# SnakeOnex/vit-is-all-you-need

Hardware: AMD Instinct MI355X
Metric: images/sec ViT-B/16 224px bf16 fwd+bwd (higher is better)
Workload: dtype bf16; 1 GPU; ViT-B/16 224x224 bf16 forward+loss+backward, batch 256 per GPU (BASELINE configs[1]; configs[2] at 8 GPUs), random-init weights, 197 tokens, 79.44 M params; global_batch=256, parallelism=dp1

## Files before the change

### vit-is-all-you-need_amd/csrc/attention.hip

```cpp
#include "common.h"

namespace {

constexpr int DH = 64;
constexpr int MAX_N = 512;
constexpr int MAX_N_LONG = 16384;
constexpr float NEG_BIG = -1.0e30f;

typedef LDS_AS bf16x4* lds_bf16x4_ptr;

__device__ __forceinline__ int swz(int row) { return (((row >> 1) & 1) << 2) | ((row >> 3) & 3); }

__device__ __forceinline__ void stage_tile(const __bf16* __restrict__ g, int ld, int N, int npad, char* lds, int wave, int lane, int nwaves = 4) {
  const int pieces = npad / 8;
  for (int pc = wave; pc < pieces; pc += nwaves) {
    const int row = pc * 8 + (lane >> 3);
    const int logical = (lane & 7) ^ swz(row);
    const int grow = min(row, N - 1);
    glds16(g + (size_t)grow * ld + logical * 8, lds + pc * 1024);
  }
}

__device__ __forceinline__ bf16x8 row_frag(const char* tile, int T, int kk, int lane) {
  const int rr = lane & 31;
// ... 361 lines not shown
  char* oimg = smem + 2 * npad * 128 + wave * 2048;
  const __bf16* qbase = a.qkv + (size_t)b * N * D3 + hh * DH;
  stage_tile(qbase + D, D3, N, npad, ktile, wave, lane, 8);
  stage_tile(qbase + 2 * D, D3, N, npad, vtile, wave, lane, 8);
  const int qb = (wave + head) & 7;
  const bool active = qb < nt;
  bf16x8 qf[4];
  load_lane_frags(qbase, D3, N, (active ? qb : 0) * 32, lane, qf);
  asm volatile("s_waitcnt vmcnt(0)" ::: "memory");
#pragma unroll
  for (int kk = 0; kk < 4; ++kk) asm volatile("" : "+v"(qf[kk]));
  __syncthreads();
  if (!active) return;
  const float c = a.scale_log2e;
  const int q0 = qb * 32;
  const int qrow = q0 + (lane & 31);
  float m = NEG_BIG, l = 0.f;
  f32x16 oacc[2];
#pragma unroll
  for (int dt = 0; dt < 2; ++dt)
#pragma unroll
    for (int r = 0; r < 16; ++r) oacc[dt][r] = 0.f;
#pragma unroll 1
  for (int T = 0; T < NKT; ++T) {
    f32x16 st;
#pragma unroll
    for (int r = 0; r < 16; ++r) st[r] = 0.f;
#pragma unroll
    for (int kk = 0; kk < 4; ++kk) st = __builtin_amdgcn_mfma_f32_32x32x16_bf16(row_frag(ktile, T, kk, lane), qf[kk], st, 0, 0, 0);
    if (32 * T + 32 > N) {
#pragma unroll
      for (int r = 0; r < 16; ++r)
        if (!(32 * T + acc_row(r, lane) < N)) st[r] = NEG_BIG;
    }
    float mt = max16(st);
    mt = fmaxf(mt, __shfl_xor(mt, 32, 64));
    const float mn = fmaxf(m, mt);
    const float alpha = fast_exp2((m - mn) * c);
    m = mn;
    const float mc = mn * c;
    float lt = 0.f;
#pragma unroll
    for (int r = 0; r < 16; ++r) {
      const float pexp = fast_exp2(__builtin_fmaf(st[r], c, -mc));
      lt += pexp;
      st[r] = pexp;
    }
    l = l * alpha + lt;
    if (T > 0) {
#pragma unroll
      for (int dt = 0; dt < 2; ++dt)
#pragma unroll
        for (int r = 0; r < 16; ++r) oacc[dt][r] *= alpha;
    }
#pragma unroll
    for (int sidx = 0; sidx < 2; ++sidx) {
      const bf16x8 pf = acc_to_frag(st, sidx);
#pragma unroll
      for (int dt = 0; dt < 2; ++dt)
        oacc[dt] = __builtin_amdgcn_mfma_f32_32x32x16_bf16(tr_frag(vtile, T, sidx, dt, lane), pf, oacc[dt], 0, 0, 0);
    }
  }
  l += __shfl_xor(l, 32, 64);
  const float mc = m * c;
  const float inv = 1.0f / l;
  if constexpr (RES)
    store_rows_T_lds2k<true>(a.o + (size_t)b * N * D + hh * DH, D, N, q0, lane, oacc, inv, oimg, a.resid_in + (size_t)b * N * D + hh * DH,
                             a.resid_out + (size_t)b * N * D + hh * DH, D);
  else
    store_rows_T_lds2k(a.o + (size_t)b * N * D + hh * DH, D, N, q0, lane, oacc, inv, oimg);
  if (lane < 32 && qrow < N) a.lse2[((size_t)b * a.H + hh) * N + qrow] = mc + log2f(l);
}

template <bool DROP, bool CAUSAL>
__global__ __launch_bounds__(256, 2) void attn_bwd_dq_kernel(const AttnArgs a) {
  extern __shared__ __attribute__((aligned(16))) char smem[];
  const int lane = threadIdx.x & 63, wave = __builtin_amdgcn_readfirstlane(threadIdx.x >> 6);
  const int b = blockIdx.x / a.H, hh = blockIdx.x % a.H;
  const int N = a.N, D3 = 3 * a.H * DH, D = a.H * DH;
  const int nt = (N + 31) / 32, npad = nt * 32;
  char* ktile = smem;
  char* vtile = smem + npad * 128;
  char* oimg = smem + 2 * npad * 128 + wave * 4096;
  const __bf16* qbase = a.qkv + (size_t)b * N * D3 + hh * DH;
  stage_tile(qbase + D, D3, N, npad, ktile, wave, lane);
  stage_tile(qbase + 2 * D, D3, N, npad, vtile, wave, lane);
  asm volatile("s_waitcnt vmcnt(0)" ::: "memory");
  __syncthreads();

  const float c = a.scale_log2e;
  const __bf16* obase = a.o + (size_t)b * N * D + hh * DH;
  const __bf16* dobase = a.d_o + (size_t)b * N * D + hh * DH;
  float csum_q = 0.f;
  for (int qb = (wave + blockIdx.x) & 3; qb < nt; qb += 4) {
    const int q0 = qb * 32;
    const int qrow = q0 + (lane & 31);
    bf16x8 qf[4], dof[4], of[4];
    load_lane_frags(qbase, D3, N, q0, lane, qf);
    load_lane_frags(dobase, D, N, q0, lane, dof);
    load_lane_frags(obase, D, N, q0, lane, of);
    float delta = 0.f;
#pragma unroll
    for (int kk = 0; kk < 4; ++kk)
#pragma unroll
      for (int j = 0; j < 8; ++j) delta += (float)dof[kk][j] * (float)of[kk][j];
    delta += __shfl_xor(delta, 32, 64);
    const size_t stat = ((size_t)b * a.H + hh) * N + min(qrow, N - 1);
    const float lse2 = a.lse2[stat];
    if (lane < 32 && qrow < N) a.delta[stat] = delta;

    f32x16 dq[2];
#pragma unroll
    for (int dt = 0; dt < 2; ++dt)
#pragma unroll
      for (int r = 0; r < 16; ++r) dq[dt][r] = 0.f;
    const int t_end = CAUSAL ? min(nt, qb + 1) : nt;
    for (int T = 0; T < t_end; ++T) {
      f32x16 s, dp;
#pragma unroll
      for (int r = 0; r < 16; ++r) { s[r] = 0.f; dp[r] = 0.f; }
#pragma unroll
      for (int kk = 0; kk < 4; ++kk) {
        s = __builtin_amdgcn_mfma_f32_32x32x16_bf16(row_frag(ktile, T, kk, lane), qf[kk], s, 0, 0, 0);
        dp = __builtin_amdgcn_mfma_f32_32x32x16_bf16(row_frag(vtile, T, kk, lane), dof[kk], dp, 0, 0, 0);
      }
#pragma unroll
      for (int r = 0; r < 16; ++r) {
        const float pexp = fast_exp2(__builtin_fmaf(s[r], c, -lse2));
        float dpr = dp[r];
        if constexpr (DROP) dpr *= attn_keep(a, blockIdx.x, min(qrow, N - 1), min(32 * T + acc_row(r, lane), N - 1));
        s[r] = pexp * (dpr - delta);
      }
      if (32 * T + 32 > N || (CAUSAL && T == qb)) {
#pragma unroll
        for (int r = 0; r < 16; ++r) {
          const int key = 32 * T + acc_row(r, lane);
          if (!(key < N && (!CAUSAL || key <= qrow))) s[r] = 0.f;
        }
      }
#pragma unroll
      for (int sidx = 0; sidx < 2; ++sidx) {
        const bf16x8 dsf = acc_to_frag(s, sidx);
#pragma unroll
        for (int dt = 0; dt < 2; ++dt)
          dq[dt] = __builtin_amdgcn_mfma_f32_32x32x16_bf16(tr_frag(ktile, T, sidx, dt, lane), dsf, dq[dt], 0, 0, 0);
      }
    }
    store_rows_T_lds(a.dqkv + (size_t)b * N * D3 + hh * DH, D3, N, q0, lane, dq, a.scale, oimg, a.dbias ? &csum_q : nullptr);
  }
  if (a.dbias) atomicAdd(a.dbias + hh * DH + lane, csum_q);
}

template <int NT>
__global__ __launch_bounds__(256, 2) void attn_bwd_dq_pipe_kernel(const AttnArgs a) {
  extern __shared__ __attribute__((aligned(16))) char smem[];
  const int lane = threadIdx.x & 63, wave = __builtin_amdgcn_readfirstlane(threadIdx.x >> 6);
  const int head = blockIdx.x;
  const int b = head / a.H, hh = head % a.H;
  const int N = a.N, D3 = 3 * a.H * DH, D = a.H * DH;
  constexpr int nt = NT, npad = NT * 32;
  char* ktile = smem;
  char* vtile = smem + npad * 128;
  char* oimg = smem + 2 * npad * 128 + wave * 4096;
  const __bf16* qbase = a.qkv + (size_t)b * N * D3 + hh * DH;
  stage_tile(qbase + D, D3, N, npad, ktile, wave, lane);
  stage_tile(qbase + 2 * D, D3, N, npad, vtile, wave, lane);
  const __bf16* obase = a.o + (size_t)b * N * D + hh * DH;
  const __bf16* dobase = a.d_o + (size_t)b * N * D + hh * DH;
  asm volatile("s_waitcnt vmcnt(0)" ::: "memory");
  __syncthreads();

  const float c = a.scale_log2e;
  float csum_q = 0.f;
  for (int qb = (wave + head) & 3; qb < nt; qb += 4) {
    const int q0 = qb * 32;
    const int qrow = q0 + (lane & 31);
    bf16x8 qf[4], dof[4];
    float delta = 0.f;
    {
      bf16x8 of[4];
      load_lane_frags(qbase, D3, N, q0, lane, qf);
      load_lane_frags(dobase, D, N, q0, lane, dof);
      load_lane_frags(obase, D, N, q0, lane, of);
#pragma unroll
      for (int kk = 0; kk < 4; ++kk)
#pragma unroll
        for (int j = 0; j < 8; ++j) delta += (float)dof[kk][j] * (float)of[kk][j];
    }
    delta += __shfl_xor(delta, 32, 64);
    const size_t stat = ((size_t)b * a.H + hh) * N + min(qrow, N - 1);
    const float lse2 = a.lse2[stat];
    if (lane < 32 && qrow < N) a.delta[stat] = delta;

    f32x16 dq[2];
#pragma unroll
    for (int dt = 0; dt < 2; ++dt)
#pragma unroll
      for (int r = 0; r < 16; ++r) dq[dt][r] = 0.f;
    bf16x8 kr[2][4], vr[2][4];
    f32x16 sb[2], dpb[2];
    auto products = [&](int buf) {
#pragma unroll
      for (int r = 0; r < 16; ++r) { sb[buf][r] = 0.f; dpb[buf][r] = 0.f; }
#pragma unroll
      for (int kk = 0; kk < 4; ++kk) {
        sb[buf] = __builtin_amdgcn_mfma_f32_32x32x16_bf16(kr[buf][kk], qf[kk], sb[buf], 0, 0, 0);
        dpb[buf] = __builtin_amdgcn_mfma_f32_32x32x16_bf16(vr[buf][kk], dof[kk], dpb[buf], 0, 0, 0);
      }
    };
#pragma unroll
    for (int kk = 0; kk < 4; ++kk) { kr[0][kk] = row_frag(ktile, 0, kk, lane); vr[0][kk] = row_frag(vtile, 0, kk, lane); }
    if (NT > 1) {
#pragma unroll
      for (int kk = 0; kk < 4; ++kk) { kr[1][kk] = row_frag(ktile, 1, kk, lane); vr[1][kk] = row_frag(vtile, 1, kk, lane); }
    }
    products(0);
#pragma unroll
    for (int T = 0; T < NT; ++T) {
      const int cur = T & 1, nxt = cur ^ 1;
      bf16x8 ktr[2][2];
#pragma unroll
      for (int sidx = 0; sidx < 2; ++sidx)
#pragma unroll
        for (int dt = 0; dt < 2; ++dt) ktr[sidx][dt] = tr_frag(ktile, T, sidx, dt, lane);
      __builtin_amdgcn_sched_barrier(0);
      if (T + 1 < NT) products(nxt);
      if (T + 2 < NT) {
#pragma unroll
        for (int kk = 0; kk < 4; ++kk) { kr[cur][kk] = row_frag(ktile, T + 2, kk, lane); vr[cur][kk] = row_frag(vtile, T + 2, kk, lane); }
      }
#pragma unroll
      for (int r = 0; r < 16; ++r) {
        const float pexp = fast_exp2(__builtin_fmaf(sb[cur][r], c, -lse2));
        sb[cur][r] = pexp * (dpb[cur][r] - delta);
      }
      if (T == NT - 1 && 32 * T + 32 > N) {
#pragma unroll
        for (int r = 0; r < 16; ++r)
          if (!(32 * T + acc_row(r, lane) < N)) sb[cur][r] = 0.f;
      }
#pragma unroll
      for (int sidx = 0; sidx < 2; ++sidx) {
        const bf16x8 dsf = acc_to_frag(sb[cur], sidx);
#pragma unroll
        for (int dt = 0; dt < 2; ++dt) dq[dt] = __builtin_amdgcn_mfma_f32_32x32x16_bf16(ktr[sidx][dt], dsf, dq[dt], 0, 0, 0);
      }
    }
    store_rows_T_lds(a.dqkv + (size_t)b * N * D3 + hh * DH, D3, N, q0, lane, dq, a.scale, oimg, a.dbias ? &csum_q : nullptr);
  }
  if (a.dbias) atomicAdd(a.dbias + hh * DH + lane, csum_q);
}

template <bool DROP, bool CAUSAL>
__global__ __launch_bounds__(256, 2) void attn_bwd_dkv_kernel(const AttnArgs a) {
  extern __shared__ __attribute__((aligned(16))) char smem[];
  const int lane = threadIdx.x & 63, wave = __builtin_amdgcn_readfirstlane(threadIdx.x >> 6);
  const int b = blockIdx.x / a.H, hh = blockIdx.x % a.H;
  const int N = a.N, D3 = 3 * a.H * DH, D = a.H * DH;
  const int nt = (N + 31) / 32, npad = nt * 32;
  char* qtile = smem;
  char* dotile = smem + npad * 128;
  float* lse_s = (float*)(smem + 2 * npad * 128);
  float* delta_s = lse_s + npad;
  char* oimg = smem + 2 * npad * 128 + 2 * npad * 4 + wave * 4096;
  const __bf16* qbase = a.qkv + (size_t)b * N * D3 + hh * DH;
  const __bf16* dobase = a.d_o + (size_t)b * N * D + hh * DH;
  stage_tile(qbase, D3, N, npad, qtile, wave, lane);
  stage_tile(dobase, D, N, npad, dotile, wave, lane);
  for (int i = threadIdx.x; i < npad; i += 256) {
    const size_t stat = ((size_t)b * a.H + hh) * N + min(i, N - 1);
    lse_s[i] = a.lse2[stat];
    delta_s[i] = a.delta[stat];
  }
  asm volatile("s_waitcnt vmcnt(0)" ::: "memory");
  __syncthreads();

  const float c = a.scale_log2e;
  float csum_k = 0.f, csum_v = 0.f;
  for (int kb = (wave + blockIdx.x) & 3; kb < nt; kb += 4) {
    const int k0 = kb * 32;
    const int krow = k0 + (lane & 31);
    bf16x8 kf[4], vf[4];
    load_lane_frags(qbase + D, D3, N, k0, lane, kf);
    load_lane_frags(qbase + 2 * D, D3, N, k0, lane, vf);
    f32x16 dk[2], dv[2];
#pragma unroll
    for (int dt = 0; dt < 2; ++dt)
#pragma unroll
      for (int r = 0; r < 16; ++r) { dk[dt][r] = 0.f; dv[dt][r] = 0.f; }
    const int t_beg = CAUSAL ? kb : 0;
    for (int T = t_beg; T < nt; ++T) {
      f32x16 s, dp;
#pragma unroll
      for (int r = 0; r < 16; ++r) { s[r] = 0.f; dp[r] = 0.f; }
#pragma unroll
      for (int kk = 0; kk < 4; ++kk) {
        s = __builtin_amdgcn_mfma_f32_32x32x16_bf16(row_frag(qtile, T, kk, lane), kf[kk], s, 0, 0, 0);
        dp = __builtin_amdgcn_mfma_f32_32x32x16_bf16(row_frag(dotile, T, kk, lane), vf[kk], dp, 0, 0, 0);
      }
      f32x16 pmat;
#pragma unroll
      for (int u = 0; u < 4; ++u) {
        const int qr = 32 * T + 8 * u + 4 * (lane >> 5);
        const f32x4 lse4 = *(const f32x4*)(lse_s + qr);
        const f32x4 del4 = *(const f32x4*)(delta_s + qr);
#pragma unroll
        for (int i = 0; i < 4; ++i) {
          const int r = 4 * u + i;
          const float pexp = fast_exp2(__builtin_fmaf(s[r], c, -lse4[i]));
          float keep = 1.0f;
          if constexpr (DROP) keep = attn_keep(a, blockIdx.x, min(qr + i, N - 1), min(krow, N - 1));
          pmat[r] = pexp * keep;
          s[r] = pexp * (dp[r] * keep - del4[i]);
        }
        if (32 * T + 32 > N || k0 + 32 > N || (CAUSAL && T == kb)) {
#pragma unroll
          for (int i = 0; i < 4; ++i) {
            const int r = 4 * u + i, query = qr + i;
            if (!(query < N && krow < N && (!CAUSAL || krow <= query))) { pmat[r] = 0.f; s[r] = 0.f; }
          }
        }
      }
#pragma unroll
      for (int sidx = 0; sidx < 2; ++sidx) {
        const bf16x8 pf = acc_to_frag(pmat, sidx);
        const bf16x8 dsf = acc_to_frag(s, sidx);
#pragma unroll
        for (int dt = 0; dt < 2; ++dt) {
          dv[dt] = __builtin_amdgcn_mfma_f32_32x32x16_bf16(tr_frag(dotile, T, sidx, dt, lane), pf, dv[dt], 0, 0, 0);
          dk[dt] = __builtin_amdgcn_mfma_f32_32x32x16_bf16(tr_frag(qtile, T, sidx, dt, lane), dsf, dk[dt], 0, 0, 0);
        }
      }
    }
    __bf16* dbase = a.dqkv + (size_t)b * N * D3 + hh * DH;
    store_rows_T_lds(dbase + D, D3, N, k0, lane, dk, a.scale, oimg, a.dbias ? &csum_k : nullptr);
    store_rows_T_lds(dbase + 2 * D, D3, N, k0, lane, dv, 1.0f, oimg, a.dbias ? &csum_v : nullptr);
  }
  if (a.dbias) {
    atomicAdd(a.dbias + D + hh * DH + lane, csum_k);
    atomicAdd(a.dbias + 2 * D + hh * DH + lane, csum_v);
  }
}

template <int NT>
__global__ __launch_bounds__(256, 2) void attn_bwd_dkv_pipe_kernel(const AttnArgs a) {
  extern __shared__ __attribute__((aligned(16))) char smem[];
  const int lane = threadIdx.x & 63, wave = __builtin_amdgcn_readfirstlane(threadIdx.x >> 6);
  const int head = blockIdx.x;
  const int b = head / a.H, hh = head % a.H;
  const int N = a.N, D3 = 3 * a.H * DH, D = a.H * DH;
  constexpr int nt = NT, npad = NT * 32;
  char* qtile = smem;
  char* dotile = smem + npad * 128;
  float* lse_s = (float*)(smem + 2 * npad * 128);
  float* delta_s = lse_s + npad;
  char* oimg = smem + 2 * npad * 128 + 2 * npad * 4 + wave * 4096;
  const __bf16* qbase = a.qkv + (size_t)b * N * D3 + hh * DH;
  const __bf16* dobase = a.d_o + (size_t)b * N * D + hh * DH;
  stage_tile(qbase, D3, N, npad, qtile, wave, lane);
  stage_tile(dobase, D, N, npad, dotile, wave, lane);
  for (int i = threadIdx.x; i < npad; i += 256) {
    const size_t stat = ((size_t)b * a.H + hh) * N + min(i, N - 1);
    lse_s[i] = i < N ? a.lse2[stat] : 1.0e30f;
    delta_s[i] = a.delta[stat];
  }
  asm volatile("s_waitcnt vmcnt(0)" ::: "memory");
  __syncthreads();

  const float c = a.scale_log2e;
  float csum_k = 0.f, csum_v = 0.f;
  for (int kb = (wave + head) & 3; kb < nt; kb += 4) {
    const int k0 = kb * 32;
    bf16x8 kf[4], vf[4];
    load_lane_frags(qbase + D, D3, N, k0, lane, kf);
    load_lane_frags(qbase + 2 * D, D3, N, k0, lane, vf);
    f32x16 dk[2], dv[2];
#pragma unroll
    for (int dt = 0; dt < 2; ++dt)
#pragma unroll
      for (int r = 0; r < 16; ++r) { dk[dt][r] = 0.f; dv[dt][r] = 0.f; }
    bf16x8 qr[4], dor[4];
    f32x16 sb, dpb;
    auto products = [&]() {
#pragma unroll
      for (int r = 0; r < 16; ++r) { sb[r] = 0.f; dpb[r] = 0.f; }
#pragma unroll
      for (int kk = 0; kk < 4; ++kk) {
        sb = __builtin_amdgcn_mfma_f32_32x32x16_bf16(qr[kk], kf[kk], sb, 0, 0, 0);
        dpb = __builtin_amdgcn_mfma_f32_32x32x16_bf16(dor[kk], vf[kk], dpb, 0, 0, 0);
      }
    };
#pragma unroll
    for (int kk = 0; kk < 4; ++kk) { qr[kk] = row_frag(qtile, 0, kk, lane); dor[kk] = row_frag(dotile, 0, kk, lane); }
    products();
    if (NT > 1) {
#pragma unroll
      for (int kk = 0; kk < 4; ++kk) { qr[kk] = row_frag(qtile, 1, kk, lane); dor[kk] = row_frag(dotile, 1, kk, lane); }
    }
#pragma unroll
    for (int T = 0; T < NT; ++T) {
      bf16x8 dotr[2][2], qtr[2][2];
      f32x4 lse4[4], del4[4];
#pragma unroll
      for (int sidx = 0; sidx < 2; ++sidx)
#pragma unroll
        for (int dt = 0; dt < 2; ++dt) { dotr[sidx][dt] = tr_frag(dotile, T, sidx, dt, lane); qtr[sidx][dt] = tr_frag(qtile, T, sidx, dt, lane); }
      __builtin_amdgcn_sched_barrier(0);
#pragma unroll
      for (int u = 0; u < 4; ++u) {
        const int qr0 = 32 * T + 8 * u + 4 * (lane >> 5);
        lse4[u] = *(const f32x4*)(lse_s + qr0);
        del4[u] = *(const f32x4*)(delta_s + qr0);
      }
      f32x16 pmat;
#pragma unroll
      for (int u = 0; u < 4; ++u)
#pragma unroll
        for (int i = 0; i < 4; ++i) {
          const int r = 4 * u + i;
          const float pexp = fast_exp2(__builtin_fmaf(sb[r], c, -lse4[u][i]));
          pmat[r] = pexp;
          sb[r] = pexp * (dpb[r] - del4[u][i]);
        }
#pragma unroll
      for (int sidx = 0; sidx < 2; ++sidx) {
        const bf16x8 pf = acc_to_frag(pmat, sidx);
        const bf16x8 dsf = acc_to_frag(sb, sidx);
#pragma unroll
        for (int dt = 0; dt < 2; ++dt) {
          dv[dt] = __builtin_amdgcn_mfma_f32_32x32x16_bf16(dotr[sidx][dt], pf, dv[dt], 0, 0, 0);
          dk[dt] = __builtin_amdgcn_mfma_f32_32x32x16_bf16(qtr[sidx][dt], dsf, dk[dt], 0, 0, 0);
        }
      }
      if (T + 1 < NT) products();
      if (T + 2 < NT) {
#pragma unroll
        for (int kk = 0; kk < 4; ++kk) { qr[kk] = row_frag(qtile, T + 2, kk, lane); dor[kk] = row_frag(dotile, T + 2, kk, lane); }
      }
    }
    __bf16* dbase = a.dqkv + (size_t)b * N * D3 + hh * DH;
    store_rows_T_lds(dbase + D, D3, N, k0, lane, dk, a.scale, oimg, a.dbias ? &csum_k : nullptr);
    store_rows_T_lds(dbase + 2 * D, D3, N, k0, lane, dv, 1.0f, oimg, a.dbias ? &csum_v : nullptr);
  }
  if (a.dbias) {
    atomicAdd(a.dbias + D + hh * DH + lane, csum_k);
    atomicAdd(a.dbias + 2 * D + hh * DH + lane, csum_v);
  }
}

constexpr int CH = 512;

template <bool DROP>
__global__ __launch_bounds__(256) void attn_fwd_long_kernel(const AttnArgs a) {
  extern __shared__ __attribute__((aligned(16))) char smem[];
  const int lane = threadIdx.x & 63, wave = __builtin_amdgcn_readfirstlane(threadIdx.x >> 6);
  const int b = blockIdx.x / a.H, hh = blockIdx.x % a.H;
  const int N = a.N, D3 = 3 * a.H * DH, D = a.H * DH;
  const int nt = (N + 31) / 32;
  char* ktile = smem;
  char* vtile = smem + CH * 128;
  const __bf16* qbase = a.qkv + (size_t)b * N * D3 + hh * DH;
  const int qb = blockIdx.y * 4 + wave;
  const bool active = qb < nt;
  const int q0 = qb * 32, qrow = q0 + (lane & 31);
  const float c = a.scale_log2e;
  bf16x8 qf[4];
  if (active) load_lane_frags(qbase, D3, N, q0, lane, qf);
  f32x16 oacc[2];
#pragma unroll
  for (int dt = 0; dt < 2; ++dt)
#pragma unroll
    for (int r = 0; r < 16; ++r) oacc[dt][r] = 0.f;
  float m = NEG_BIG, l = 0.f;
  const int t_end = a.causal ? min(nt, qb + 1) : nt;
  for (int k0 = 0; k0 < N; k0 += CH) {
    const int rows = min(CH, N - k0), ntc = (rows + 31) / 32;
    __syncthreads();
    stage_tile(qbase + D + (size_t)k0 * D3, D3, rows, ntc * 32, ktile, wave, lane);
    stage_tile(qbase + 2 * D + (size_t)k0 * D3, D3, rows, ntc * 32, vtile, wave, lane);
    asm volatile("s_waitcnt vmcnt(0)" ::: "memory");
    __syncthreads();
    if (!active) continue;
    for (int T = 0; T < ntc && k0 / 32 + T < t_end; ++T) {
      const int key0 = k0 + 32 * T;
      f32x16 s;
#pragma unroll
      for (int r = 0; r < 16; ++r) s[r] = 0.f;
#pragma unroll
      for (int kk = 0; kk < 4; ++kk) s = __builtin_amdgcn_mfma_f32_32x32x16_bf16(row_frag(ktile, T, kk, lane), qf[kk], s, 0, 0, 0);
      if (key0 + 32 > N || (a.causal && key0 / 32 == qb)) {
#pragma unroll
        for (int r = 0; r < 16; ++r) {
          const int key = key0 + acc_row(r, lane);
          if (!(key < N && (!a.causal || key <= qrow))) s[r] = NEG_BIG;
        }
      }
      float tmax = max16(s);
      tmax = fmaxf(tmax, __shfl_xor(tmax, 32, 64)) * c;
      const float mnew = fmaxf(m, tmax);
      const float alpha = fast_exp2(m - mnew);
      m = mnew;
      float psum = 0.f;
#pragma unroll
      for (int r = 0; r < 16; ++r) {
        s[r] = fast_exp2(__builtin_fmaf(s[r], c, -mnew));
        psum += s[r];
        if constexpr (DROP) s[r] *= attn_keep(a, blockIdx.x, min(qrow, N - 1), min(key0 + acc_row(r, lane), N - 1));
      }
      l = l * alpha + psum;
#pragma unroll
      for (int dt = 0; dt < 2; ++dt)
#pragma unroll
        for (int r = 0; r < 16; ++r) oacc[dt][r] *= alpha;
#pragma unroll
      for (int sidx = 0; sidx < 2; ++sidx) {
        const bf16x8 pf = acc_to_frag(s, sidx);
#pragma unroll
        for (int dt = 0; dt < 2; ++dt)
          oacc[dt] = __builtin_amdgcn_mfma_f32_32x32x16_bf16(tr_frag(vtile, T, sidx, dt, lane), pf, oacc[dt], 0, 0, 0);
      }
    }
  }
  if (!active) return;
  l += __shfl_xor(l, 32, 64);
  const float inv = 1.0f / l;
  store_rows_T(a.o + (size_t)b * N * D + hh * DH, D, N, q0, lane, oacc, inv);
  if (lane < 32 && qrow < N) a.lse2[((size_t)b * a.H + hh) * N + qrow] = m + log2f(l);
}

template <bool DROP>
__global__ __launch_bounds__(256) void attn_bwd_dq_long_kernel(const AttnArgs a) {
  extern __shared__ __attribute__((aligned(16))) char smem[];
  const int lane = threadIdx.x & 63, wave = __builtin_amdgcn_readfirstlane(threadIdx.x >> 6);
  const int b = blockIdx.x / a.H, hh = blockIdx.x % a.H;
  const int N = a.N, D3 = 3 * a.H * DH, D = a.H * DH;
  const int nt = (N + 31) / 32;
  char* ktile = smem;
  char* vtile = smem + CH * 128;
  char* oimg = smem + 2 * CH * 128 + wave * 4096;
  const __bf16* qbase = a.qkv + (size_t)b * N * D3 + hh * DH;
  const __bf16* obase = a.o + (size_t)b * N * D + hh * DH;
  const __bf16* dobase = a.d_o + (size_t)b * N * D + hh * DH;
  const int qb = blockIdx.y * 4 + wave;
  const bool active = qb < nt;
  const int q0 = qb * 32, qrow = q0 + (lane & 31);
  const float c = a.scale_log2e;
  bf16x8 qf[4], dof[4];
  float delta = 0.f, lse2 = 0.f;
  if (active) {
    bf16x8 of[4];
    load_lane_frags(qbase, D3, N, q0, lane, qf);
    load_lane_frags(dobase, D, N, q0, lane, dof);
    load_lane_frags(obase, D, N, q0, lane, of);
#pragma unroll
    for (int kk = 0; kk < 4; ++kk)
#pragma unroll
      for (int j = 0; j < 8; ++j) delta += (float)dof[kk][j] * (float)of[kk][j];
    delta += __shfl_xor(delta, 32, 64);
    const size_t stat = ((size_t)b * a.H + hh) * N + min(qrow, N - 1);
    lse2 = a.lse2[stat];
    if (lane < 32 && qrow < N) a.delta[stat] = delta;
  }
  f32x16 dq[2];
#pragma unroll
  for (int dt = 0; dt < 2; ++dt)
#pragma unroll
    for (int r = 0; r < 16; ++r) dq[dt][r] = 0.f;
  const int t_end = a.causal ? min(nt, qb + 1) : nt;
  for (int k0 = 0; k0 < N; k0 += CH) {
    const int rows = min(CH, N - k0), ntc = (rows + 31) / 32;
    __syncthreads();
    stage_tile(qbase + D + (size_t)k0 * D3, D3, rows, ntc * 32, ktile, wave, lane);
    stage_tile(qbase + 2 * D + (size_t)k0 * D3, D3, rows, ntc * 32, vtile, wave, lane);
    asm volatile("s_waitcnt vmcnt(0)" ::: "memory");
    __syncthreads();
    if (!active) continue;
    for (int T = 0; T < ntc && k0 / 32 + T < t_end; ++T) {
      const int key0 = k0 + 32 * T;
      f32x16 s, dp;
#pragma unroll
      for (int r = 0; r < 16; ++r) { s[r] = 0.f; dp[r] = 0.f; }
#pragma unroll
      for (int kk = 0; kk < 4; ++kk) {
        s = __builtin_amdgcn_mfma_f32_32x32x16_bf16(row_frag(ktile, T, kk, lane), qf[kk], s, 0, 0, 0);
        dp = __builtin_amdgcn_mfma_f32_32x32x16_bf16(row_frag(vtile, T, kk, lane), dof[kk], dp, 0, 0, 0);
      }
#pragma unroll
      for (int r = 0; r < 16; ++r) {
        const float pexp = fast_exp2(__builtin_fmaf(s[r], c, -lse2));
        float dpr = dp[r];
        if constexpr (DROP) dpr *= attn_keep(a, blockIdx.x, min(qrow, N - 1), min(key0 + acc_row(r, lane), N - 1));
        s[r] = pexp * (dpr - delta);
      }
      if (key0 + 32 > N || (a.causal && key0 / 32 == qb)) {
#pragma unroll
        for (int r = 0; r < 16; ++r) {
          const int key = key0 + acc_row(r, lane);
          if (!(key < N && (!a.causal || key <= qrow))) s[r] = 0.f;
        }
      }
// ... 90 lines not shown
#pragma unroll
      for (int sidx = 0; sidx < 2; ++sidx) {
        const bf16x8 pf = acc_to_frag(pmat, sidx);
        const bf16x8 dsf = acc_to_frag(s, sidx);
#pragma unroll
        for (int dt = 0; dt < 2; ++dt) {
          dv[dt] = __builtin_amdgcn_mfma_f32_32x32x16_bf16(tr_frag(dotile, T, sidx, dt, lane), pf, dv[dt], 0, 0, 0);
          dk[dt] = __builtin_amdgcn_mfma_f32_32x32x16_bf16(tr_frag(qtile, T, sidx, dt, lane), dsf, dk[dt], 0, 0, 0);
        }
      }
    }
  }
  if (!active) return;
  float csum_k = 0.f, csum_v = 0.f;
  __bf16* dbase = a.dqkv + (size_t)b * N * D3 + hh * DH;
  store_rows_T_lds(dbase + D, D3, N, k0, lane, dk, a.scale, oimg, a.dbias ? &csum_k : nullptr);
  store_rows_T_lds(dbase + 2 * D, D3, N, k0, lane, dv, 1.0f, oimg, a.dbias ? &csum_v : nullptr);
  if (a.dbias) {
    atomicAdd(a.dbias + D + hh * DH + lane, csum_k);
    atomicAdd(a.dbias + 2 * D + hh * DH + lane, csum_v);
  }
}

int check(const AttnArgs& a) {
  if (a.B <= 0 || a.N <= 0 || a.H <= 0 || a.N > MAX_N_LONG) return VITAMD_ERR_SHAPE;
  return VITAMD_OK;
}

}

static bool attn_dropout(AttnArgs& a, float p, unsigned long long seed) {
  if (!(p >= 0.f) || p >= 1.f) return false;
  a.drop_thresh = p > 0.f ? (unsigned)((double)p * 4294967296.0) : 0u;
  if (p > 0.f && a.drop_thresh == 0u) a.drop_thresh = 1u;
  a.drop_scale = 1.0f / (1.0f - p);
  a.seed_lo = (unsigned)seed;
  a.seed_hi = (unsigned)(seed >> 32);
  return true;
}

template <int K, bool DROP, bool CAUSAL>
static int launch_fwd_small_c(const AttnArgs& a, int lds, hipStream_t stream) {
  if (a.resid_in) {
    if (int e = set_lds((attn_fwd_small_kernel<K, DROP, CAUSAL, true>), lds)) return e;
    hipLaunchKernelGGL((attn_fwd_small_kernel<K, DROP, CAUSAL, true>), dim3(a.B * a.H), dim3(256), lds, stream, a);
    return VITAMD_OK;
  }
  if (int e = set_lds((attn_fwd_small_kernel<K, DROP, CAUSAL>), lds)) return e;
  hipLaunchKernelGGL((attn_fwd_small_kernel<K, DROP, CAUSAL>), dim3(a.B * a.H), dim3(256), lds, stream, a);
  return VITAMD_OK;
}
template <int K, bool DROP>
static int launch_fwd_small(const AttnArgs& a, int lds, hipStream_t stream) {
  return a.causal ? launch_fwd_small_c<K, DROP, true>(a, lds, stream) : launch_fwd_small_c<K, DROP, false>(a, lds, stream);
}

static int attention_fwd_impl(const void* qkv, void* o, float* lse2, const float* resid_in, float* resid_out, int B, int N, int H,
                              int head_dim, int causal, float dropout_p, unsigned long long seed, void* stream_);

extern "C" int vitamd_attention_fwd(const void* qkv, void* o, float* lse2, int B, int N, int H, int head_dim, int causal,
                                    float dropout_p, unsigned long long seed, void* stream_) {
  return attention_fwd_impl(qkv, o, lse2, nullptr, nullptr, B, N, H, head_dim, causal, dropout_p, seed, stream_);
}

extern "C" int vitamd_attention_fwd_resid(const void* qkv, void* o, float* lse2, const float* resid_in, float* resid_out, int B, int N,
                                          int H, int head_dim, int causal, float dropout_p, unsigned long long seed, void* stream_) {
  if (!resid_in || !resid_out) return VITAMD_ERR_ARG;
  if (N > 256) return VITAMD_ERR_SHAPE;
  return attention_fwd_impl(qkv, o, lse2, resid_in, resid_out, B, N, H, head_dim, causal, dropout_p, seed, stream_);
}

static int attention_fwd_impl(const void* qkv, void* o, float* lse2, const float* resid_in, float* resid_out, int B, int N, int H,
                              int head_dim, int causal, float dropout_p, unsigned long long seed, void* stream_) {
  hipStream_t stream = (hipStream_t)stream_;
  if (head_dim != DH) return VITAMD_ERR_SHAPE;
  AttnArgs a{(const __bf16*)qkv, (__bf16*)o, lse2, nullptr, nullptr, nullptr, nullptr, B, N, H, causal, 0.125f * 1.4426950408889634f, 0.125f,
             0u, 1.0f, 0u, 0u, resid_in, resid_out};
  if (int e = check(a)) return e;
  if (!qkv || !o || !lse2 || !attn_dropout(a, dropout_p, seed)) return VITAMD_ERR_ARG;
  const bool drop = a.drop_thresh != 0u;
  const int nkt = (N + 31) / 32, npad = nkt * 32;
  if (N > MAX_N) {
    const int lds = 2 * CH * 128;
    const dim3 grid(B * H, (nkt + 3) / 4);
    if (drop) {
      if (int e = set_lds(attn_fwd_long_kernel<true>, lds)) return e;
      hipLaunchKernelGGL(attn_fwd_long_kernel<true>, grid, dim3(256), lds, stream, a);
    } else {
      if (int e = set_lds(attn_fwd_long_kernel<false>, lds)) return e;
      hipLaunchKernelGGL(attn_fwd_long_kernel<false>, grid, dim3(256), lds, stream, a);
    }
    return hipGetLastError() == hipSuccess ? VITAMD_OK : VITAMD_ERR_LAUNCH;
  }
  if (nkt >= 5 && nkt <= 8 && !drop && !causal) {
    const int lds = 2 * npad * 128 + 8 * 2048;
    int e = VITAMD_OK;
#define FWD_SMALL8(K) case K: \
      if (a.resid_in) { e = set_lds(attn_fwd_small8_kernel<K, true>, lds); if (!e) hipLaunchKernelGGL((attn_fwd_small8_kernel<K, true>), dim3(B * H), dim3(512), lds, stream, a); } \
      else { e = set_lds(attn_fwd_small8_kernel<K, false>, lds); if (!e) hipLaunchKernelGGL((attn_fwd_small8_kernel<K, false>), dim3(B * H), dim3(512), lds, stream, a); } break;
    switch (nkt) { FWD_SMALL8(5) FWD_SMALL8(6) FWD_SMALL8(7) FWD_SMALL8(8) }
#undef FWD_SMALL8
    if (e) return e;
  } else if (nkt <= 8) {
    const int lds = 2 * npad * 128 + 4 * 4096;
    int e = VITAMD_OK;
#define FWD_SMALL(K) case K: e = drop ? launch_fwd_small<K, true>(a, lds, stream) : launch_fwd_small<K, false>(a, lds, stream); break;
    switch (nkt) { FWD_SMALL(1) FWD_SMALL(2) FWD_SMALL(3) FWD_SMALL(4) FWD_SMALL(5) FWD_SMALL(6) FWD_SMALL(7) FWD_SMALL(8) }
#undef FWD_SMALL
    if (e) return e;
  } else {
    const int lds = 2 * npad * 128;
    if (drop) {
      if (int e = set_lds(attn_fwd_kernel<true>, lds)) return e;
      hipLaunchKernelGGL(attn_fwd_kernel<true>, dim3(B * H), dim3(256), lds, stream, a);
    } else {
      if (int e = set_lds(attn_fwd_kernel<false>, lds)) return e;
      hipLaunchKernelGGL(attn_fwd_kernel<false>, dim3(B * H), dim3(256), lds, stream, a);
    }
  }
  return hipGetLastError() == hipSuccess ? VITAMD_OK : VITAMD_ERR_LAUNCH;
}

extern "C" int vitamd_attention_bwd(const void* qkv, const void* o, const float* lse2, const void* d_o, void* dqkv, float* delta,
                                    float* dbias, int B, int N, int H, int head_dim, int causal, float dropout_p,
                                    unsigned long long seed, void* stream_) {
  hipStream_t stream = (hipStream_t)stream_;
  if (head_dim != DH) return VITAMD_ERR_SHAPE;
  AttnArgs a{(const __bf16*)qkv, (__bf16*)o, (float*)lse2, (const __bf16*)d_o, (__bf16*)dqkv, delta, dbias, B, N, H, causal,
             0.125f * 1.4426950408889634f, 0.125f, 0u, 1.0f, 0u, 0u, nullptr, nullptr};
  if (int e = check(a)) return e;
  if (!qkv || !o || !lse2 || !d_o || !dqkv || !delta || !attn_dropout(a, dropout_p, seed)) return VITAMD_ERR_ARG;
  if (N > MAX_N) {
    const int ldsq = 2 * CH * 128 + 4 * 4096, ldsk = 2 * CH * 128 + 2 * CH * 4 + 4 * 4096;
    const dim3 grid(B * H, ((N + 31) / 32 + 3) / 4);
    if (a.drop_thresh) {
      if (int e = set_lds(attn_bwd_dq_long_kernel<true>, ldsq)) return e;
      if (int e = set_lds(attn_bwd_dkv_long_kernel<true>, ldsk)) return e;
      hipLaunchKernelGGL(attn_bwd_dq_long_kernel<true>, grid, dim3(256), ldsq, stream, a);
      hipLaunchKernelGGL(attn_bwd_dkv_long_kernel<true>, grid, dim3(256), ldsk, stream, a);
    } else {
      if (int e = set_lds(attn_bwd_dq_long_kernel<false>, ldsq)) return e;
      if (int e = set_lds(attn_bwd_dkv_long_kernel<false>, ldsk)) return e;
      hipLaunchKernelGGL(attn_bwd_dq_long_kernel<false>, grid, dim3(256), ldsq, stream, a);
      hipLaunchKernelGGL(attn_bwd_dkv_long_kernel<false>, grid, dim3(256), ldsk, stream, a);
    }
    return hipGetLastError() == hipSuccess ? VITAMD_OK : VITAMD_ERR_LAUNCH;
  }
  const int npad = (N + 31) / 32 * 32;
  const int lds1 = 2 * npad * 128 + 4 * 4096, lds2 = 2 * npad * 128 + 2 * npad * 4 + 4 * 4096;
  const dim3 grid(B * H), block(256);
  const int nkt = npad / 32;
  if (!a.drop_thresh && !a.causal && nkt >= 2 && nkt <= 7) {
    int e = VITAMD_OK;
#define DQ_PIPE(K) case K: e = set_lds(attn_bwd_dq_pipe_kernel<K>, lds1); if (!e) hipLaunchKernelGGL(attn_bwd_dq_pipe_kernel<K>, grid, block, lds1, stream, a); break;
    switch (nkt) { DQ_PIPE(2) DQ_PIPE(3) DQ_PIPE(4) DQ_PIPE(5) DQ_PIPE(6) DQ_PIPE(7) }
#undef DQ_PIPE
    if (e) return e;
#define DKV_PIPE(K) case K: e = set_lds(attn_bwd_dkv_pipe_kernel<K>, lds2); if (!e) hipLaunchKernelGGL(attn_bwd_dkv_pipe_kernel<K>, grid, block, lds2, stream, a); break;
    switch (nkt) { DKV_PIPE(2) DKV_PIPE(3) DKV_PIPE(4) DKV_PIPE(5) DKV_PIPE(6) DKV_PIPE(7) }
#undef DKV_PIPE
    if (e) return e;
    return hipGetLastError() == hipSuccess ? VITAMD_OK : VITAMD_ERR_LAUNCH;
  }
#define BWD_SMALL(DROP, CAUSAL)                                                                      \
  do {                                                                                               \
    if (int e = set_lds((attn_bwd_dq_kernel<DROP, CAUSAL>), lds1)) return e;                         \
    if (int e = set_lds((attn_bwd_dkv_kernel<DROP, CAUSAL>), lds2)) return e;                        \
    hipLaunchKernelGGL((attn_bwd_dq_kernel<DROP, CAUSAL>), grid, block, lds1, stream, a);  \
    hipLaunchKernelGGL((attn_bwd_dkv_kernel<DROP, CAUSAL>), grid, block, lds2, stream, a);          \
  } while (0)
  if (a.drop_thresh) { if (a.causal) BWD_SMALL(true, true); else BWD_SMALL(true, false); }
  else { if (a.causal) BWD_SMALL(false, true); else BWD_SMALL(false, false); }
#undef BWD_SMALL
  return hipGetLastError() == hipSuccess ? VITAMD_OK : VITAMD_ERR_LAUNCH;
}
```

### vit-is-all-you-need_amd/vitamd/ops.py

```python
from __future__ import annotations

import torch

from . import lib as _lib

EPI_BIAS_BF16, EPI_GELU, EPI_RESID_F32, EPI_DGELU, EPI_PATCH_F32, EPI_F32, EPI_GELU_DG, EPI_DMUL = range(8)
import os as _os
NT_PERSISTENT = _os.environ.get("VITAMD_NT_PERSISTENT", "1") != "0"
_seam_env = _os.environ.get("VITAMD_NT_SEAM", "auto")
NT_SEAM = {"1": True, "0": False}.get(_seam_env)
SEAM_PROBE = {}
NT_FORM_SEAM, NT_FORM_LOADER = 4, 5
_RAW_AUTO = -1
LN_EPS = 1e-5
BF16, F32 = torch.bfloat16, torch.float32


def _L():
    return _lib.load()


_INITIALISED = set()


# ... 85 lines not shown
    for name, tile in (("seam_us", _RAW_AUTO), ("plain_us", 1024)):
        launch = lambda: gemm_nt(x, w, EPI_BIAS_BF16, out=out, tile=tile)
        launch()
        s, e = torch.cuda.Event(enable_timing=True), torch.cuda.Event(enable_timing=True)
        s.record()
        for _ in range(reps):
            launch()
        e.record()
        e.synchronize()
        times[name] = s.elapsed_time(e) / reps * 1e3
    on = times["seam_us"] <= 1.25 * times["plain_us"]
    SEAM_PROBE[device.index] = {"seam_us": round(times["seam_us"], 1), "plain_us": round(times["plain_us"], 1), "enabled": on}
    if not on:
        import warnings
        warnings.warn(f"vitamd: the seam form of the NT GEMM is slower than the plain persistent form on {device} "
                      f"({times['seam_us']:.0f} vs {times['plain_us']:.0f} us): switched off for this device")
    return on


_WORKSPACES = {}


def _workspace(device, nbytes):
    key = (device, torch.cuda.current_stream().cuda_stream)
    ws = _WORKSPACES.get(key)
    if ws is None or ws.numel() * 4 < nbytes:
        ws = _WORKSPACES[key] = torch.empty((nbytes + 3) // 4, dtype=F32, device=device)
    return ws


TN_FORM_SHARED, TN_FORM_EXCLUSIVE = 0, 1


def gemm_tn(l, r, out, splits=0, accumulate=True, atomic=False, form=TN_FORM_SHARED):
    _need(l, BF16, "l", 2); _need(r, BF16, "r", 2); _need(out, F32, "out", 2)
    R, P = l.shape
    R2, Q = r.shape
    if R != R2 or tuple(out.shape) != (P, Q):
        raise _lib.VitamdError("gemm_tn: shape mismatch")
    if atomic:
        if not accumulate:
            raise _lib.VitamdError("gemm_tn: the atomic form can only accumulate")
        code = _L().vitamd_gemm_tn_bf16(_p(l), _p(r), _p(out), R, P, Q, P, Q, Q, splits, _stream())
    else:
        nbytes = _L().vitamd_gemm_tn_ws_bytes(R, P, Q, splits)
        ws = _workspace(l.device, nbytes)
        code = _L().vitamd_gemm_tn_bf16_ws(_p(l), _p(r), _p(out), R, P, Q, P, Q, Q, splits, _p(ws), ws.numel() * 4, int(accumulate),
                                           int(form), _stream())
    _lib.check(code, f"gemm_tn[R={R},P={P},Q={Q}]")
    return out


def layernorm_fwd(x, addend=None):
    _need(x, F32, "x", 2)
    M, D = x.shape
    y = torch.empty((M, D), dtype=BF16, device=x.device)
    mean = torch.empty((M,), dtype=F32, device=x.device)
    rstd = torch.empty((M,), dtype=F32, device=x.device)
    x_out = None
    if addend is not None:
        _need(addend, BF16, "addend", 2)
        x_out = torch.empty_like(x)
    code = _L().vitamd_layernorm_fwd(_p(x), _p(addend), _p(x_out), _p(y), _p(mean), _p(rstd), M, D, LN_EPS, _stream())
    _lib.check(code, f"layernorm_fwd[M={M},D={D}]")
    return (x_out if addend is not None else x), y, mean, rstd


def layernorm_bwd(dy, x, mean, rstd, g_res=None, want_bf16=False, colsum=None, dropout=(0.0, 0), xhat=None):
    _need(dy, BF16, "dy", 2); _need(x, F32, "x", 2)
    M, D = x.shape
    g = torch.empty_like(x)
    gb = torch.empty((M, D), dtype=BF16, device=x.device) if want_bf16 else None
    if g_res is not None:
        _need(g_res, F32, "g_res", 2)
    if xhat is not None and D in (256, 512, 768, 1024):
        _need(xhat, BF16, "xhat", 2)
        code = _L().vitamd_layernorm_bwd_xhat(_p(dy), _p(xhat), _p(rstd), _p(g_res), _p(g), _p(gb), _p(colsum), M, D,
                                              float(dropout[0]), int(dropout[1]), _stream())
        _lib.check(code, f"layernorm_bwd_xhat[M={M},D={D}]")
        return g, gb
    code = _L().vitamd_layernorm_bwd_dropout(_p(dy), _p(x), _p(mean), _p(rstd), _p(g_res), _p(g), _p(gb), _p(colsum), M, D,
                                             float(dropout[0]), int(dropout[1]), _stream())
    _lib.check(code, f"layernorm_bwd[M={M},D={D}]")
    return g, gb


def layernorm_affine_fwd(x, gamma, beta, eps=LN_EPS):
    _need(x, F32, "x", 2); _need(gamma, F32, "gamma", 1); _need(beta, F32, "beta", 1)
    M, D = x.shape
    y = torch.empty((M, D), dtype=BF16, device=x.device)
    mean = torch.empty((M,), dtype=F32, device=x.device)
    rstd = torch.empty((M,), dtype=F32, device=x.device)
    _lib.check(_L().vitamd_layernorm_affine_fwd(_p(x), _p(gamma), _p(beta), _p(y), _p(mean), _p(rstd), M, D, float(eps), _stream()),
               "layernorm_affine_fwd")
    return y, mean, rstd


def layernorm_affine_bwd(dy, x, mean, rstd, gamma, dgamma, dbeta, g_res=None, want_bf16=False, colsum=None):
    _need(dy, BF16, "dy", 2); _need(x, F32, "x", 2); _need(gamma, F32, "gamma", 1)
    _need(dgamma, F32, "dgamma", 1); _need(dbeta, F32, "dbeta", 1)
    M, D = x.shape
    g = torch.empty_like(x)
    gb = torch.empty((M, D), dtype=BF16, device=x.device) if want_bf16 else None
    _lib.check(_L().vitamd_layernorm_affine_bwd(_p(dy), _p(x), _p(mean), _p(rstd), _p(gamma), _p(g_res), _p(g), _p(gb), _p(colsum),
                                                _p(dgamma), _p(dbeta), M, D, _stream()), "layernorm_affine_bwd")
    return g, gb


def layernorm_affine_fwd_f32(x, gamma, beta, eps=LN_EPS):
    _need(x, F32, "x", 2); _need(gamma, F32, "gamma", 1); _need(beta, F32, "beta", 1)
    M, D = x.shape
    y = torch.empty_like(x)
    mean = torch.empty((M,), dtype=F32, device=x.device)
    rstd = torch.empty((M,), dtype=F32, device=x.device)
    _lib.check(_L().vitamd_layernorm_affine_fwd_f32(_p(x), _p(gamma), _p(beta), _p(y), _p(mean), _p(rstd), M, D, float(eps), _stream()),
               "layernorm_affine_fwd_f32")
    return y, mean, rstd


def layernorm_affine_bwd_f32(dy, x, mean, rstd, gamma, dgamma, dbeta):
    _need(dy, F32, "dy", 2); _need(x, F32, "x", 2); _need(gamma, F32, "gamma", 1)
    _need(dgamma, F32, "dgamma", 1); _need(dbeta, F32, "dbeta", 1)
    M, D = x.shape
    g = torch.empty_like(x)
    _lib.check(_L().vitamd_layernorm_affine_bwd_f32(_p(dy), _p(x), _p(mean), _p(rstd), _p(gamma), _p(g), _p(dgamma), _p(dbeta), M, D,
                                                    _stream()), "layernorm_affine_bwd_f32")
    return g


ATTN_RESID_MAX_N = 256


def attention_fwd(qkv, B, N, H, causal=False, dropout=(0.0, 0), resid=None):
    _need(qkv, BF16, "qkv", 2)
    D = H * 64
    if tuple(qkv.shape) != (B * N, 3 * D):
        raise _lib.VitamdError("attention_fwd: qkv must be [B*N, 3*H*64] (head_dim 64 only)")
    o = torch.empty((B * N, D), dtype=BF16, device=qkv.device)
    lse = torch.empty((B, H, N), dtype=F32, device=qkv.device)
    if resid is not None:
        _need(resid, F32, "resid", 2)
        if tuple(resid.shape) != (B * N, D):
            raise _lib.VitamdError("attention_fwd: resid must be [B*N, H*64]")
        x1 = torch.empty_like(resid)
        code = _L().vitamd_attention_fwd_resid(_p(qkv), _p(o), _p(lse), _p(resid), _p(x1), B, N, H, 64, int(causal), float(dropout[0]),
                                               int(dropout[1]), _stream())
        _lib.check(code, f"attention_fwd_resid[B={B},N={N},H={H}]")
        return o, lse, x1
    code = _L().vitamd_attention_fwd(_p(qkv), _p(o), _p(lse), B, N, H, 64, int(causal), float(dropout[0]), int(dropout[1]), _stream())
    _lib.check(code, f"attention_fwd[B={B},N={N},H={H}]")
    return o, lse


def attention_bwd(qkv, o, lse, d_o, B, N, H, causal=False, dbias=None, dropout=(0.0, 0)):
    _need(qkv, BF16, "qkv", 2); _need(o, BF16, "o", 2); _need(d_o, BF16, "d_o", 2); _need(lse, F32, "lse")
    if dbias is not None:
        _need(dbias, F32, "dbias", 1)
    dqkv = torch.empty_like(qkv)
    delta = torch.empty_like(lse)
    code = _L().vitamd_attention_bwd(_p(qkv), _p(o), _p(lse), _p(d_o), _p(dqkv), _p(delta), _p(dbias), B, N, H, 64, int(causal),
                                     float(dropout[0]), int(dropout[1]), _stream())
    _lib.check(code, f"attention_bwd[B={B},N={N},H={H}]")
    return dqkv


def linear_dropout_resid(a, b, bias, resid, dropout):
    _need(a, BF16, "a", 2); _need(b, BF16, "b", 2); _need(resid, F32, "resid", 2); _need(bias, F32, "bias", 1)
    M, K = a.shape
    N = b.shape[0]
    out = torch.empty((M, N), dtype=F32, device=a.device)
    code = _L().vitamd_linear_dropout_resid_bf16(_p(a), _p(b), _p(out), _p(bias), _p(resid), M, N, K, float(dropout[0]), int(dropout[1]),
                                                 0 if NT_PERSISTENT else 512, _stream())
    _lib.check(code, f"linear_dropout_resid[M={M},N={N},K={K}]")
    return out


def cast_bf16_dropout(x, dropout):
    _need(x, F32, "x")
    out = torch.empty(x.shape, dtype=BF16, device=x.device)
    _lib.check(_L().vitamd_cast_f32_bf16_dropout(_p(x), _p(out), x.numel(), float(dropout[0]), int(dropout[1]), _stream()), "cast_dropout")
    return out


def dropout(x, p, seed, group=1, inplace=False):
    if x.dtype not in (BF16, F32):
        raise _lib.VitamdError(f"dropout: expected bf16 or fp32, got {x.dtype}")
    _need(x, x.dtype, "x")
    out = x if inplace else torch.empty_like(x)
    fn = _L().vitamd_dropout_bf16 if x.dtype == BF16 else _L().vitamd_dropout_f32
    _lib.check(fn(_p(x), _p(out), x.numel(), int(group), float(p), int(seed), _stream()), "dropout")
    return out


def cast_bf16(x):
    _need(x, F32, "x")
    out = torch.empty(x.shape, dtype=BF16, device=x.device)
    _lib.check(_L().vitamd_cast_f32_bf16(_p(x), _p(out), x.numel(), _stream()), "cast_f32_bf16")
    return out


def cast_weight(w, want_plain=True, want_transposed=False):
    _need(w, F32, "w", 2)
    N, K = w.shape
    wb = torch.empty((N, K), dtype=BF16, device=w.device) if want_plain else None
    wbt = torch.empty((K, N), dtype=BF16, device=w.device) if want_transposed else None
    _lib.check(_L().vitamd_cast_transpose_weight(_p(w), _p(wb), _p(wbt), N, K, _stream()), "cast_transpose_weight")
    return wb, wbt


def im2col(img, p):
    _need(img, F32, "img", 4)
    B, C, H, W = img.shape
    out = torch.empty((B * (H // p) * (W // p), C * p * p), dtype=BF16, device=img.device)
    _lib.check(_L().vitamd_im2col_bf16(_p(img), _p(out), B, C, H, W, p, _stream()), "im2col")
    return out


def colsum(x, out=None):
    _need(x, BF16, "x", 2)
    M, N = x.shape
    if out is None:
        out = torch.zeros((N,), dtype=F32, device=x.device)
    _lib.check(_L().vitamd_colsum_bf16(_p(x), _p(out), M, N, N, _stream()), "colsum")
    return out


def embed_bwd(g, B, seq, extra, D):
    _need(g, F32, "g", 2)
    n_p = seq - extra
    dev = g.device
    dpos = torch.zeros((n_p, D), dtype=F32, device=dev)
    dextra = torch.zeros((extra, D), dtype=F32, device=dev)
    dyp = torch.empty((B * n_p, D), dtype=BF16, device=dev)
    dbias = torch.zeros((D,), dtype=F32, device=dev)
    rows = torch.zeros((max(n_p, 1), D), dtype=F32, device=dev)
    _lib.check(_L().vitamd_embed_bwd(_p(g), _p(dpos), _p(dextra) if extra > 0 else None, _p(dyp), _p(dbias), _p(rows), B, seq, extra, D,
                                     _stream()), "embed_bwd")
    return dpos, dextra, dyp, dbias


def vq_nearest(x, codebook):
    _need(x, F32, "x", 2); _need(codebook, F32, "codebook", 2)
    M, d = x.shape
    K, d2 = codebook.shape
    if d != d2:
        raise _lib.VitamdError("vq_nearest: dim mismatch")
    idx = torch.empty((M,), dtype=torch.int64, device=x.device)
    _lib.check(_L().vitamd_vq_nearest(_p(x), _p(codebook), _p(idx), M, K, d, _stream()), "vq_nearest")
    return idx


def conv3x3_fwd(x, w, bias):
    _need(x, F32, "x", 4); _need(w, F32, "w", 4)
    B, C, H, W = x.shape
    Co = w.shape[0]
    if tuple(w.shape) != (Co, C, 3, 3):
        raise _lib.VitamdError("conv3x3: weight must be [Cout, Cin, 3, 3]")
    y = torch.empty((B, Co, H, W), dtype=F32, device=x.device)
    _lib.check(_L().vitamd_conv3x3_fwd(_p(x), _p(w), _p(bias), _p(y), B, C, Co, H, W, _stream()), f"conv3x3_fwd[Cin={C},Cout={Co}]")
    return y


def conv3x3_bwd(x, w, dy, need_dx=True, need_dw=True, has_bias=True):
    _need(x, F32, "x", 4); _need(w, F32, "w", 4); _need(dy, F32, "dy", 4)
    B, C, H, W = x.shape
    Co = w.shape[0]
    if tuple(dy.shape) != (B, Co, H, W):
        raise _lib.VitamdError("conv3x3_bwd: dy shape mismatch")
    dx = torch.empty_like(x) if need_dx else None
    dw = torch.zeros_like(w) if need_dw else None
    db = torch.zeros((Co,), dtype=F32, device=x.device) if (need_dw and has_bias) else None
    _lib.check(_L().vitamd_conv3x3_bwd(_p(x), _p(w), _p(dy), _p(dx), _p(dw), _p(db), B, C, Co, H, W, _stream()), "conv3x3_bwd")
    return dx, dw, db


SKINNY_MAX_M = 64
SKINNY_EPIS = (EPI_BIAS_BF16, EPI_GELU, EPI_RESID_F32, EPI_F32)
DECODE_MAX_LEN = 16384


def _need_len(length):
    _need(length, torch.int32, "len")
    if length.numel() != 1:
        raise _lib.VitamdError("len: expected a one-element device int32")
    return length


def _need_cache(k_cache, v_cache, B, H):
    _need(k_cache, BF16, "k_cache", 4); _need(v_cache, BF16, "v_cache", 4)
    if k_cache.shape != v_cache.shape or k_cache.shape[0] != B or k_cache.shape[1] != H or k_cache.shape[3] != 64:
        raise _lib.VitamdError(f"cache: expected k and v bf16 [B={B}, H={H}, Lmax, 64], got {tuple(k_cache.shape)} / {tuple(v_cache.shape)}")
    Lmax = k_cache.shape[2]
    if not 1 <= Lmax <= DECODE_MAX_LEN:
        raise _lib.VitamdError(f"cache: Lmax must be in [1, {DECODE_MAX_LEN}], got {Lmax}")
    return Lmax


def kv_append(qkv, k_cache, v_cache, length, B, T, H, host_len=None):
    _need(qkv, BF16, "qkv", 2); _need_len(length)
    Lmax = _need_cache(k_cache, v_cache, B, H)
    if tuple(qkv.shape) != (B * T, 3 * H * 64):
        raise _lib.VitamdError(f"kv_append: qkv must be [B*T, 3*H*64] = [{B * T}, {3 * H * 64}], got {tuple(qkv.shape)}")
    if T > Lmax or (host_len is not None and host_len + T > Lmax):
        raise _lib.VitamdError(f"kv_append: len {host_len} + T {T} exceeds the cache length {Lmax}")
    _lib.check(_L().vitamd_kv_append(_p(qkv), _p(k_cache), _p(v_cache), _p(length), B, T, H, 64, Lmax, _stream()),
               f"kv_append[B={B},T={T},H={H},Lmax={Lmax}]")


def decode_attention(qkv, k_cache, v_cache, length, B, H, host_len=None):
    _need(qkv, BF16, "qkv", 2); _need_len(length)
    Lmax = _need_cache(k_cache, v_cache, B, H)
    if tuple(qkv.shape) != (B, 3 * H * 64):
# ... 47 lines not shown
```

Baseline: 8740 images/sec.

## Merge attention backward dQ and dKV pipe kernels into one paired launch

Turns the dQ and dKV pipelined backward kernels into device bodies and dispatches both from a single kernel. Blocks are grouped so that each chunk of 64 heads has its dQ blocks followed by its dKV blocks, which lets the two halves run concurrently and removes one launch. The dKV body now recomputes delta (rowsum of dO·O) itself instead of reading it from global memory, which removes the dependency on a delta buffer written elsewhere. The cost is extra loads of O and dO per block and LDS sized to the larger of the two kernels. ops.py also gains an optional caller-supplied delta buffer.

```diff
diff --git a/vit-is-all-you-need_amd/csrc/attention.hip b/vit-is-all-you-need_amd/csrc/attention.hip
--- a/vit-is-all-you-need_amd/csrc/attention.hip
+++ b/vit-is-all-you-need_amd/csrc/attention.hip
@@ -537,10 +537,8 @@
 }
 
 template <int NT>
-__global__ __launch_bounds__(256, 2) void attn_bwd_dq_pipe_kernel(const AttnArgs a) {
-  extern __shared__ __attribute__((aligned(16))) char smem[];
+__device__ __forceinline__ void attn_bwd_dq_pipe_body(const AttnArgs& a, char* smem, const int head) {
   const int lane = threadIdx.x & 63, wave = __builtin_amdgcn_readfirstlane(threadIdx.x >> 6);
-  const int head = blockIdx.x;
   const int b = head / a.H, hh = head % a.H;
   const int N = a.N, D3 = 3 * a.H * DH, D = a.H * DH;
   constexpr int nt = NT, npad = NT * 32;
@@ -728,10 +726,8 @@
 }
 
 template <int NT>
-__global__ __launch_bounds__(256, 2) void attn_bwd_dkv_pipe_kernel(const AttnArgs a) {
-  extern __shared__ __attribute__((aligned(16))) char smem[];
+__device__ __forceinline__ void attn_bwd_dkv_pipe_body(const AttnArgs& a, char* smem, const int head) {
   const int lane = threadIdx.x & 63, wave = __builtin_amdgcn_readfirstlane(threadIdx.x >> 6);
-  const int head = blockIdx.x;
   const int b = head / a.H, hh = head % a.H;
   const int N = a.N, D3 = 3 * a.H * DH, D = a.H * DH;
   constexpr int nt = NT, npad = NT * 32;
@@ -747,7 +743,22 @@
   for (int i = threadIdx.x; i < npad; i += 256) {
     const size_t stat = ((size_t)b * a.H + hh) * N + min(i, N - 1);
     lse_s[i] = i < N ? a.lse2[stat] : 1.0e30f;
-    delta_s[i] = a.delta[stat];
+  }
+  {
+    const __bf16* obase = a.o + (size_t)b * N * D + hh * DH;
+    for (int qb = wave; qb < nt; qb += 4) {
+      const int q0 = qb * 32;
+      bf16x8 dof[4], of[4];
+      float delta = 0.f;
+      load_lane_frags(dobase, D, N, q0, lane, dof);
+      load_lane_frags(obase, D, N, q0, lane, of);
+#pragma unroll
+      for (int kk = 0; kk < 4; ++kk)
+#pragma unroll
+        for (int j = 0; j < 8; ++j) delta += (float)dof[kk][j] * (float)of[kk][j];
+      delta += __shfl_xor(delta, 32, 64);
+      if (lane < 32) delta_s[q0 + lane] = delta;
+    }
   }
   asm volatile("s_waitcnt vmcnt(0)" ::: "memory");
   __syncthreads();
@@ -831,6 +842,17 @@
     atomicAdd(a.dbias + D + hh * DH + lane, csum_k);
     atomicAdd(a.dbias + 2 * D + hh * DH + lane, csum_v);
   }
+}
+
+constexpr int PAIR_HEADS = 64;
+
+template <int NT>
+__global__ __launch_bounds__(256, 2) void attn_bwd_pair_kernel(const AttnArgs a) {
+  extern __shared__ __attribute__((aligned(16))) char smem[];
+  const int id = blockIdx.x, base = id / (2 * PAIR_HEADS) * PAIR_HEADS;
+  const int nb = min(PAIR_HEADS, a.B * a.H - base), r = id - 2 * base;
+  if (r < nb) attn_bwd_dq_pipe_body<NT>(a, smem, base + r);
+  else attn_bwd_dkv_pipe_body<NT>(a, smem, base + r - nb);
 }
 
 constexpr int CH = 512;
@@ -1227,13 +1249,10 @@
   const int nkt = npad / 32;
   if (!a.drop_thresh && !a.causal && nkt >= 2 && nkt <= 7) {
     int e = VITAMD_OK;
-#define DQ_PIPE(K) case K: e = set_lds(attn_bwd_dq_pipe_kernel<K>, lds1); if (!e) hipLaunchKernelGGL(attn_bwd_dq_pipe_kernel<K>, grid, block, lds1, stream, a); break;
-    switch (nkt) { DQ_PIPE(2) DQ_PIPE(3) DQ_PIPE(4) DQ_PIPE(5) DQ_PIPE(6) DQ_PIPE(7) }
-#undef DQ_PIPE
-    if (e) return e;
-#define DKV_PIPE(K) case K: e = set_lds(attn_bwd_dkv_pipe_kernel<K>, lds2); if (!e) hipLaunchKernelGGL(attn_bwd_dkv_pipe_kernel<K>, grid, block, lds2, stream, a); break;
-    switch (nkt) { DKV_PIPE(2) DKV_PIPE(3) DKV_PIPE(4) DKV_PIPE(5) DKV_PIPE(6) DKV_PIPE(7) }
-#undef DKV_PIPE
+    const int ldsp = lds1 > lds2 ? lds1 : lds2;
+#define BWD_PAIR(K) case K: e = set_lds(attn_bwd_pair_kernel<K>, ldsp); if (!e) hipLaunchKernelGGL(attn_bwd_pair_kernel<K>, dim3(2 * B * H), block, ldsp, stream, a); break;
+    switch (nkt) { BWD_PAIR(2) BWD_PAIR(3) BWD_PAIR(4) BWD_PAIR(5) BWD_PAIR(6) BWD_PAIR(7) }
+#undef BWD_PAIR
     if (e) return e;
     return hipGetLastError() == hipSuccess ? VITAMD_OK : VITAMD_ERR_LAUNCH;
   }
diff --git a/vit-is-all-you-need_amd/vitamd/ops.py b/vit-is-all-you-need_amd/vitamd/ops.py
--- a/vit-is-all-you-need_amd/vitamd/ops.py
+++ b/vit-is-all-you-need_amd/vitamd/ops.py
@@ -261,12 +261,17 @@
     return o, lse
 
 
-def attention_bwd(qkv, o, lse, d_o, B, N, H, causal=False, dbias=None, dropout=(0.0, 0)):
+def attention_bwd(qkv, o, lse, d_o, B, N, H, causal=False, dbias=None, dropout=(0.0, 0), delta=None):
     _need(qkv, BF16, "qkv", 2); _need(o, BF16, "o", 2); _need(d_o, BF16, "d_o", 2); _need(lse, F32, "lse")
     if dbias is not None:
         _need(dbias, F32, "dbias", 1)
     dqkv = torch.empty_like(qkv)
-    delta = torch.empty_like(lse)
+    if delta is None:
+        delta = torch.empty_like(lse)
+    else:
+        _need(delta, F32, "delta")
+        if tuple(delta.shape) != tuple(lse.shape):
+            raise _lib.VitamdError("attention_bwd: delta must be fp32 [B, H, N]")
     code = _L().vitamd_attention_bwd(_p(qkv), _p(o), _p(lse), _p(d_o), _p(dqkv), _p(delta), _p(dbias), B, N, H, 64, int(causal),
                                      float(dropout[0]), int(dropout[1]), _stream())
     _lib.check(code, f"attention_bwd[B={B},N={N},H={H}]")
```

Result: no change. 8771 images/sec (median of 6 runs) (+0.4%).
